# razorx89/nmfgpu

Measured on AMD Instinct MI355X. Metric: NMF MU iterations/sec, dense 10kx5k r=64, higher is better.
Workload: dtype f32; 1 GPU; configs[1]: dense random V 10000x5000, r=64, MU Frobenius, fp32; rows=10000, columns=5000, features=64, error_every=10, parallelism=single GPU

## Files before the change

nmfgpu_amd/csrc/kernels_mu64.hip:

```cpp
#include <hip/hip_runtime.h>
#include <stdint.h>

#include "kernels.h"
#include "split3.h"
#include "gram_image.h"

namespace nmfamd {

typedef float f32x16 __attribute__((ext_vector_type(16)));

template <bool IS_W>
__global__ __launch_bounds__(256) void k_mu64_update(
	float* __restrict__ P, const float* __restrict__ slabs, int S, long slab_stride,
	const float* __restrict__ Q, const float* __restrict__ scale, float eps,
	float* __restrict__ ps, int len_valid, float* __restrict__ gram_partial,
	const float* __restrict__ Gprev, int compute_error, bf16x8* __restrict__ x3_out, int x3_ks) {
	__shared__ __attribute__((aligned(16))) float s_num[64][68];
	__shared__ __attribute__((aligned(16))) float s_old[64][68];
	__shared__ float s_ps[2][64];
	const int tid = threadIdx.x;
	const int wave = tid >> 6, lane = tid & 63;
	const int half = lane >> 5, l31 = lane & 31;
	const int ct = wave & 1, mb = wave >> 1;
	const long tile = (long)blockIdx.x * 64 * 64;
	const int c4 = (4 * tid) & 63;
	const int yl0 = tid >> 4;

	f32x4 nl[4], ol[4];
	{
		f32x4 t[7][4];
#pragma unroll
		for (int j = 0; j < 4; ++j) {
			const long e = tile + 4 * (tid + 256 * j);
			nl[j] = *reinterpret_cast<const f32x4*>(slabs + e);
			ol[j] = *reinterpret_cast<const f32x4*>(P + e);
#pragma unroll
			for (int u = 0; u < 7; ++u) {
				const int k = 1 + u < S ? 1 + u : 0;
				t[u][j] = *reinterpret_cast<const f32x4*>(slabs + (long)k * slab_stride + e);
			}
		}
#pragma unroll
		for (int u = 0; u < 7; ++u)
			if (1 + u < S) {
#pragma unroll
				for (int j = 0; j < 4; ++j) nl[j] += t[u][j];
			}
		for (int k0 = 8; k0 < S; k0 += 7) {
#pragma unroll
			for (int j = 0; j < 4; ++j)
#pragma unroll
				for (int u = 0; u < 7; ++u) {
					const int k = k0 + u < S ? k0 + u : 0;
					t[u][j] = *reinterpret_cast<const f32x4*>(slabs + (long)k * slab_stride + tile + 4 * (tid + 256 * j));
				}
#pragma unroll
			for (int u = 0; u < 7; ++u)
				if (k0 + u < S) {
#pragma unroll
					for (int j = 0; j < 4; ++j) nl[j] += t[u][j];
				}
		}
	}
	const f32x4 sc = *reinterpret_cast<const f32x4*>(scale + c4);
	float qa[32];
#pragma unroll
	for (int cb = 0; cb < 2; ++cb)
#pragma unroll
		for (int q = 0; q < 4; ++q)
#pragma unroll
			for (int gi = 0; gi < 4; ++gi) qa[cb * 16 + q * 4 + gi] = Q[(long)(32 * cb + 8 * q + 4 * half + gi) * 64 + 32 * mb + l31];
#pragma unroll
	for (int j = 0; j < 4; ++j) {
		if (IS_W) ol[j] *= sc; else nl[j] *= sc;
		*reinterpret_cast<f32x4*>(&s_num[yl0 + 16 * j][c4]) = nl[j];
		*reinterpret_cast<f32x4*>(&s_old[yl0 + 16 * j][c4]) = ol[j];
	}
	__syncthreads();

	const int yrow = ct * 32 + l31;
	f32x4 oldv[2][4], numv[4];
#pragma unroll
	for (int cb = 0; cb < 2; ++cb)
#pragma unroll
		for (int q = 0; q < 4; ++q) oldv[cb][q] = *reinterpret_cast<const f32x4*>(&s_old[yrow][32 * cb + 8 * q + 4 * half]);
#pragma unroll
	for (int q = 0; q < 4; ++q) numv[q] = *reinterpret_cast<const f32x4*>(&s_num[yrow][32 * mb + 8 * q + 4 * half]);
	f32x16 acc;
#pragma unroll
	for (int g = 0; g < 16; ++g) acc[g] = 0.f;
#pragma unroll
	for (int cb = 0; cb < 2; ++cb)
#pragma unroll
		for (int q = 0; q < 4; ++q)
#pragma unroll
			for (int gi = 0; gi < 4; ++gi)
				acc = __builtin_amdgcn_mfma_f32_32x32x2f32(qa[cb * 16 + q * 4 + gi], oldv[cb][q][gi], acc, 0, 0, 0);

	float psum = 0.f;
#pragma unroll
	for (int q = 0; q < 4; ++q) {
		f32x4 o;
#pragma unroll
		for (int gi = 0; gi < 4; ++gi) {
			const float old = mb == 0 ? oldv[0][q][gi] : oldv[1][q][gi];
			o[gi] = old * numv[q][gi] / (acc[4 * q + gi] + eps);
			psum += o[gi] * numv[q][gi];
		}
		*reinterpret_cast<f32x4*>(&s_num[yrow][32 * mb + 8 * q + 4 * half]) = o;
	}
	if (!IS_W && compute_error) {
		psum += __shfl_xor(psum, 32);
		if (half == 0) s_ps[mb][yrow] = psum;
	}
	if (IS_W && compute_error && blockIdx.x == 0) {
		for (int d = wave * 16; d < wave * 16 + 16; ++d) {
			float v = Q[(long)lane * 64 + d] * Gprev[(long)d * 64 + lane];
			for (int w = 32; w > 0; w >>= 1) v += __shfl_xor(v, w);
			if (lane == 0) ps[d] = v;
		}
	}
	__syncthreads();
	if (!IS_W && compute_error && tid < 64) {
		const int ycol = blockIdx.x * 64 + tid;
		if (ycol < len_valid) ps[ycol] = s_ps[0][tid] + s_ps[1][tid];
	}

#pragma unroll
	for (int j = 0; j < 4; ++j)
		*reinterpret_cast<f32x4*>(P + tile + 4 * (tid + 256 * j)) = *reinterpret_cast<const f32x4*>(&s_num[yl0 + 16 * j][c4]);
	if (x3_out != nullptr) {
#pragma unroll
		for (int i = 0; i < 2; ++i) {
			const int slot = tid + 256 * i;
			const int r = slot & 31, h = (slot >> 5) & 1, nb = (slot >> 6) & 1, kk = slot >> 7;
			const long ks = 4l * blockIdx.x + kk;
			if (ks < x3_ks) {
				float v[8];
#pragma unroll
				for (int j = 0; j < 8; ++j) {
					const int yl = 16 * kk + 8 * h + j;
					v[j] = blockIdx.x * 64 + yl < len_valid ? s_num[yl][32 * nb + r] : 0.f;
				}
				store_split3(x3_out, ks, 2, nb, h, r, v);
			}
		}
	}
	const int ab = wave >> 1, bb = wave & 1;
	f32x16 g;
#pragma unroll
	for (int i = 0; i < 16; ++i) g[i] = 0.f;
#pragma unroll 8
	for (int x = 0; x < 64; x += 2) {
		const float a = s_num[x + half][ab * 32 + l31];
		const float b = s_num[x + half][bb * 32 + l31];
		g = __builtin_amdgcn_mfma_f32_32x32x2f32(a, b, g, 0, 0, 0);
	}
	float* out = gram_partial + (long)blockIdx.x * 4096;
#pragma unroll
	for (int q = 0; q < 4; ++q)
#pragma unroll
		for (int gi = 0; gi < 4; ++gi) out[(long)(ab * 32 + gi + 8 * q + 4 * half) * 64 + bb * 32 + l31] = g[4 * q + gi];
}

hipError_t launch_mu64_update(int is_w, float* P, const float* slabs, int S, long slab_stride, const float* Q, const float* scale,
                              float eps, float* ps, int len_valid, int len_pad, float* gram_partial, const float* Gprev,
                              int compute_error, hipStream_t stream, void* x3_out, int x3_ks) {
	dim3 grid(len_pad / 64), block(256);
	bf16x8* xo = reinterpret_cast<bf16x8*>(x3_out);
	if (is_w) hipLaunchKernelGGL((k_mu64_update<true>), grid, block, 0, stream, P, slabs, S, slab_stride, Q, scale, eps, ps, len_valid, gram_partial, Gprev, compute_error, xo, x3_ks);
	else hipLaunchKernelGGL((k_mu64_update<false>), grid, block, 0, stream, P, slabs, S, slab_stride, Q, scale, eps, ps, len_valid, gram_partial, Gprev, compute_error, xo, x3_ks);
	return hipGetLastError();
}

#ifndef U32_Q_EARLY
#define U32_Q_EARLY 0
#endif
template <bool IS_W, int U = 7, int QS = 1, bool NS = false>
__global__ __launch_bounds__(256) void k_mu64_update32(
	float* __restrict__ P, const float* __restrict__ slabs, int S, long slab_stride,
	const float* __restrict__ Q, const float* __restrict__ scale, float eps,
	float* __restrict__ ps, int len_valid, const float* __restrict__ Gprev, int compute_error, bf16x8* __restrict__ x3_out, int x3_ks, PeerSlabs peers,
	float* __restrict__ colsq_part, int qsplit, float* __restrict__ q_out, float ns_a_arg, float ns_b_arg, int ns_r) {
	static_assert(!(NS && IS_W), "the smoothing matrix rides the H update only");
	typedef float f32x4v __attribute__((ext_vector_type(4)));
	__shared__ __attribute__((aligned(16))) float s_num[32][68];
	__shared__ __attribute__((aligned(16))) float s_old[32][68];
	__shared__ __attribute__((aligned(16))) float s_sm[NS ? 32 : 1][68];
	__shared__ float s_ps[4][32];
	__shared__ float s_dsum[NS ? 4 : 1][32], s_osum[NS ? 4 : 1][32];
	const float ns_a = NS ? in_vgpr(ns_a_arg) : 1.f, ns_b = NS ? in_vgpr(ns_b_arg) : 0.f;
	const int tid = threadIdx.x;
	const int wave = tid >> 6, lane = tid & 63;
	const int q = lane >> 4, l15 = lane & 15;
	const long tile = (long)blockIdx.x * 32 * 64;
	const int c4 = (4 * tid) & 63;
	const int yl0 = tid >> 4;

	if (peers.count > 0) S = peers.count;
	if (peers.count > 1) __builtin_amdgcn_fence(__ATOMIC_ACQUIRE, "");
	auto slab_at = [&](int k) -> const float* { return peers.count > 0 ? peers.p[k] : slabs + (long)k * slab_stride; };
	f32x4v qa[4];
	f32x4v qs[QS > 1 ? QS - 1 : 1][4];
	f32x4v nl[2], ol[2];
	{
		f32x4v t[U][2];
#pragma unroll
		for (int j = 0; j < 2; ++j) {
			const long e = tile + 4 * (tid + 256 * j);
			nl[j] = *reinterpret_cast<const f32x4v*>(slab_at(0) + e);
			ol[j] = *reinterpret_cast<const f32x4v*>(P + e);
#pragma unroll
			for (int u = 0; u < U; ++u) {
				const int k = 1 + u < S ? 1 + u : 0;
				t[u][j] = *reinterpret_cast<const f32x4v*>(slab_at(k) + e);
			}
		}
		if (QS > 1 || U32_Q_EARLY) {
			__builtin_amdgcn_sched_barrier(0);
#pragma unroll
			for (int u = 0; u < 4; ++u) qa[u] = *reinterpret_cast<const f32x4v*>(Q + (long)(16 * wave + l15) * 64 + 16 * q + 4 * u);
#pragma unroll
			for (int k = 1; k < QS; ++k)
#pragma unroll
				for (int u = 0; u < 4; ++u) qs[k - 1][u] = *reinterpret_cast<const f32x4v*>(Q + (long)k * 4096 + (long)(16 * wave + l15) * 64 + 16 * q + 4 * u);
			__builtin_amdgcn_sched_barrier(0);
		}
#pragma unroll
		for (int u = 0; u < U; ++u)
			if (1 + u < S) {
#pragma unroll
				for (int j = 0; j < 2; ++j) nl[j] += t[u][j];
			}
		for (int k0 = 1 + U; k0 < S; k0 += U) {
#pragma unroll
			for (int j = 0; j < 2; ++j)
#pragma unroll
				for (int u = 0; u < U; ++u) {
					const int k = k0 + u < S ? k0 + u : 0;
					t[u][j] = *reinterpret_cast<const f32x4v*>(slab_at(k) + tile + 4 * (tid + 256 * j));
				}
#pragma unroll
			for (int u = 0; u < U; ++u)
				if (k0 + u < S) {
#pragma unroll
					for (int j = 0; j < 2; ++j) nl[j] += t[u][j];
				}
		}
	}
	const f32x4v sc = *reinterpret_cast<const f32x4v*>(scale + c4);
	if (QS == 1 && !U32_Q_EARLY) {
#pragma unroll
		for (int u = 0; u < 4; ++u) qa[u] = *reinterpret_cast<const f32x4v*>(Q + (long)(16 * wave + l15) * 64 + 16 * q + 4 * u);
	}
	if (!IS_W && QS > 1) {
#pragma unroll
		for (int k = 1; k < QS; ++k)
#pragma unroll
			for (int u = 0; u < 4; ++u) qa[u] += qs[k - 1][u];
		const float srow = scale[16 * wave + l15];
#pragma unroll
		for (int u = 0; u < 4; ++u) {
			const f32x4v scol = *reinterpret_cast<const f32x4v*>(scale + 16 * q + 4 * u);
			qa[u] = (qa[u] * scol) * srow;
			if (blockIdx.x == 0 && q_out != nullptr) *reinterpret_cast<f32x4v*>(q_out + (long)(16 * wave + l15) * 64 + 16 * q + 4 * u) = qa[u];
		}
	}
#pragma unroll
	for (int j = 0; j < 2; ++j) {
		if (IS_W) ol[j] *= sc; else nl[j] *= sc;
		if (NS) {
			float sn = (nl[j][0] + nl[j][1]) + (nl[j][2] + nl[j][3]);
			float so = (ol[j][0] + ol[j][1]) + (ol[j][2] + ol[j][3]);
#pragma unroll
			for (int w = 1; w < 16; w <<= 1) { sn += __shfl_xor(sn, w); so += __shfl_xor(so, w); }
			f32x4v sm;
#pragma unroll
			for (int g = 0; g < 4; ++g) {
				const bool in = c4 + g < ns_r;
				nl[j][g] = in ? ns_a * nl[j][g] + ns_b * sn : 0.f;
				sm[g] = in ? ns_a * ol[j][g] + ns_b * so : 0.f;
			}
			*reinterpret_cast<f32x4v*>(&s_sm[yl0 + 16 * j][c4]) = sm;
		}
		*reinterpret_cast<f32x4v*>(&s_num[yl0 + 16 * j][c4]) = nl[j];
		*reinterpret_cast<f32x4v*>(&s_old[yl0 + 16 * j][c4]) = ol[j];
	}
	__syncthreads();

	f32x4v ob[2][4];
#pragma unroll
	for (int yt = 0; yt < 2; ++yt)
#pragma unroll
		for (int u = 0; u < 4; ++u) ob[yt][u] = *reinterpret_cast<const f32x4v*>(NS ? &s_sm[16 * yt + l15][16 * q + 4 * u] : &s_old[16 * yt + l15][16 * q + 4 * u]);
	f32x4v acc[2] = {{0.f, 0.f, 0.f, 0.f}, {0.f, 0.f, 0.f, 0.f}};
#pragma unroll
	for (int u = 0; u < 4; ++u)
#pragma unroll
		for (int g = 0; g < 4; ++g) {
			acc[0] = __builtin_amdgcn_mfma_f32_16x16x4f32(qa[u][g], ob[0][u][g], acc[0], 0, 0, 0);
			acc[1] = __builtin_amdgcn_mfma_f32_16x16x4f32(qa[u][g], ob[1][u][g], acc[1], 0, 0, 0);
		}
	f32x4v sq = {0.f, 0.f, 0.f, 0.f};
	if (NS) {
#pragma unroll
		for (int yt = 0; yt < 2; ++yt) {
			float v = (acc[yt][0] + acc[yt][1]) + (acc[yt][2] + acc[yt][3]);
			v += __shfl_xor(v, 16);
			v += __shfl_xor(v, 32);
			if (q == 0) s_dsum[wave][16 * yt + l15] = v;
		}
		__syncthreads();
#pragma unroll
		for (int yt = 0; yt < 2; ++yt) {
			const int y = 16 * yt + l15;
			const float tsum = ((s_dsum[0][y] + s_dsum[1][y]) + s_dsum[2][y]) + s_dsum[3][y];
#pragma unroll
			for (int g = 0; g < 4; ++g) acc[yt][g] = ns_a * acc[yt][g] + ns_b * tsum;
		}
	}
#pragma unroll
	for (int yt = 0; yt < 2; ++yt) {
		const int y = 16 * yt + l15;
		const f32x4v oldv = *reinterpret_cast<const f32x4v*>(&s_old[y][16 * wave + 4 * q]);
		const f32x4v numv = *reinterpret_cast<const f32x4v*>(&s_num[y][16 * wave + 4 * q]);
		f32x4v o;
		float psum = 0.f;
#pragma unroll
		for (int g = 0; g < 4; ++g) {
			o[g] = oldv[g] * numv[g] / (acc[yt][g] + eps);
			psum += o[g] * numv[g];
			if (IS_W) sq[g] += o[g] * o[g];
		}
		*reinterpret_cast<f32x4v*>(&s_num[y][16 * wave + 4 * q]) = o;
		if (NS) {
			float v = (o[0] + o[1]) + (o[2] + o[3]);
			v += __shfl_xor(v, 16);
			v += __shfl_xor(v, 32);
			if (q == 0) s_osum[wave][y] = v;
		}
		if (!IS_W && compute_error) {
			psum += __shfl_xor(psum, 16);
			psum += __shfl_xor(psum, 32);
			if (q == 0) s_ps[wave][y] = psum;
		}
	}
	if (IS_W && colsq_part != nullptr) {
#pragma unroll
		for (int g = 0; g < 4; ++g) {
			float v = sq[g];
			v += __shfl_xor(v, 1); v += __shfl_xor(v, 2); v += __shfl_xor(v, 4); v += __shfl_xor(v, 8);
			sq[g] = v;
		}
		if (l15 == 0) *reinterpret_cast<f32x4v*>(colsq_part + (long)blockIdx.x * 64 + 16 * wave + 4 * q) = sq;
	}
	if (IS_W && compute_error && wave == 0) {
		for (int d = blockIdx.x; d < 64; d += gridDim.x) {
			float v = Q[(long)lane * 64 + d] * Gprev[(long)d * 64 + lane];
			for (int w = 32; w > 0; w >>= 1) v += __shfl_xor(v, w);
			if (lane == 0) ps[d] = v;
		}
	}
	__syncthreads();
	if (!IS_W && compute_error && tid < 32) {
		const int ycol = blockIdx.x * 32 + tid;
		if (ycol < len_valid) ps[ycol] = ((s_ps[0][tid] + s_ps[1][tid]) + s_ps[2][tid]) + s_ps[3][tid];
	}
#pragma unroll
	for (int j = 0; j < 2; ++j)
		*reinterpret_cast<f32x4v*>(P + tile + 4 * (tid + 256 * j)) = *reinterpret_cast<const f32x4v*>(&s_num[yl0 + 16 * j][c4]);
	{
		const int r = tid & 31, h = (tid >> 5) & 1, nb = (tid >> 6) & 1, kk = tid >> 7;
		const long ks = 2l * blockIdx.x + kk;
		if (ks < x3_ks) {
			float v[8];
#pragma unroll
			for (int j = 0; j < 8; ++j) {
				const int yl = 16 * kk + 8 * h + j;
				float x = s_num[yl][32 * nb + r];
				if (NS) x = 32 * nb + r < ns_r ? ns_a * x + ns_b * (((s_osum[0][yl] + s_osum[1][yl]) + s_osum[2][yl]) + s_osum[3][yl]) : 0.f;
				v[j] = blockIdx.x * 32 + yl < len_valid ? x : 0.f;
			}
			store_split3(x3_out, ks, 2, nb, h, r, v);
		}
	}
}

template <bool IS_W, int U, int QS, bool NS = false>
static void launch_update32_inst(dim3 grid, hipStream_t stream, float* P, const float* slabs, int S, long slab_stride, const float* Q, const float* scale, float eps, float* ps,
                                 int len_valid, const float* Gprev, int compute_error, bf16x8* xo, int x3_ks, const PeerSlabs& peers, float* colsq_part, float* q_out,
                                 const SmoothAround* ns = nullptr) {
	hipLaunchKernelGGL((k_mu64_update32<IS_W, U, QS, NS>), grid, dim3(256), 0, stream, P, slabs, S, slab_stride, Q, scale, eps, ps, len_valid, Gprev, compute_error, xo, x3_ks, peers,
	                   colsq_part, QS, q_out, NS ? ns->diag - ns->off : 1.f, NS ? ns->off : 0.f, NS ? ns->r : 0);
}

hipError_t launch_mu64_update32(int is_w, float* P, const float* slabs, int S, long slab_stride, const float* Q, const float* scale,
                                float eps, float* ps, int len_valid, int len_pad, const float* Gprev, int compute_error, hipStream_t stream,
                                void* x3_out, int x3_ks, const PeerSlabs* peers, float* colsq_part, int qsplit, float* q_out, const SmoothAround* ns) {
	if (x3_out == nullptr || len_pad % 32 != 0 || (qsplit > 1 && is_w) || (qsplit > 1 && qsplit != 2 && qsplit != 4 && qsplit != 8)) return hipErrorInvalidValue;
	if (ns != nullptr && (is_w || ns->r < 1 || ns->r > 64)) return hipErrorInvalidValue;
	PeerSlabs pa = {};
	if (peers != nullptr) {
		if (peers->count < 1 || peers->count > PEER_SLABS_MAX) return hipErrorInvalidValue;
		pa = *peers;
		S = peers->count;
	}
	dim3 grid(len_pad / 32);
	bf16x8* xo = reinterpret_cast<bf16x8*>(x3_out);
#define NMFAMD_U32(ISW, UU, QQ) launch_update32_inst<ISW, UU, QQ>(grid, stream, P, slabs, S, slab_stride, Q, scale, eps, ps, len_valid, Gprev, compute_error, xo, x3_ks, pa, colsq_part, q_out)
#define NMFAMD_U32NS(UU, QQ) launch_update32_inst<false, UU, QQ, true>(grid, stream, P, slabs, S, slab_stride, Q, scale, eps, ps, len_valid, Gprev, compute_error, xo, x3_ks, pa, colsq_part, q_out, ns)
	if (ns != nullptr) {
		if (S > 8) { if (qsplit == 2) NMFAMD_U32NS(13, 2); else if (qsplit == 4) NMFAMD_U32NS(13, 4); else if (qsplit == 8) NMFAMD_U32NS(13, 8); else NMFAMD_U32NS(13, 1); }
		else { if (qsplit == 2) NMFAMD_U32NS(7, 2); else if (qsplit == 4) NMFAMD_U32NS(7, 4); else if (qsplit == 8) NMFAMD_U32NS(7, 8); else NMFAMD_U32NS(7, 1); }
#undef NMFAMD_U32NS
		return hipGetLastError();
	}
	if (is_w) { if (S > 8) NMFAMD_U32(true, 13, 1); else NMFAMD_U32(true, 7, 1); }
	else if (S > 8) { if (qsplit == 2) NMFAMD_U32(false, 13, 2); else if (qsplit == 4) NMFAMD_U32(false, 13, 4); else if (qsplit == 8) NMFAMD_U32(false, 13, 8); else NMFAMD_U32(false, 13, 1); }
	else { if (qsplit == 2) NMFAMD_U32(false, 7, 2); else if (qsplit == 4) NMFAMD_U32(false, 7, 4); else if (qsplit == 8) NMFAMD_U32(false, 7, 8); else NMFAMD_U32(false, 7, 1); }
#undef NMFAMD_U32
	return hipGetLastError();
}

__global__ __launch_bounds__(256) void k_sum_peers(PeerSlabs src, float* __restrict__ out, int count) {
	__builtin_amdgcn_fence(__ATOMIC_ACQUIRE, "");
	const int i = 4 * (blockIdx.x * 256 + threadIdx.x);
	if (i >= count) return;
	f32x4 s = *reinterpret_cast<const f32x4*>(src.p[0] + i);
	for (int k = 1; k < src.count; ++k) s += *reinterpret_cast<const f32x4*>(src.p[k] + i);
	*reinterpret_cast<f32x4*>(out + i) = s;
}

hipError_t launch_sum_peers(const PeerSlabs& src, float* out, int count, hipStream_t stream) {
	if (src.count < 1 || src.count > PEER_SLABS_MAX || count % 4 != 0) return hipErrorInvalidValue;
	hipLaunchKernelGGL(k_sum_peers, dim3((unsigned)((count / 4 + 255) / 256)), dim3(256), 0, stream, src, out, count);
	return hipGetLastError();
}

__global__ __launch_bounds__(256) void k_gram_image(GramReduceArgs rg) {
	__shared__ __attribute__((aligned(16))) float lds[GRAM_IMAGE_LDS_FLOATS];
	gram_image_block(rg, blockIdx.x, lds);
}

hipError_t launch_gram_image_args(const GramReduceArgs& rg, hipStream_t stream) {
	if (rg.image == nullptr || rg.ksplit > GRAM_KSPLIT_MAX || (rg.ksplit > 1 && rg.normalize != 0 && rg.colsq_part == nullptr)) return hipErrorInvalidValue;
	hipLaunchKernelGGL(k_gram_image, dim3(rg.ksplit > 1 ? GRAM_IMAGE_TILES * rg.ksplit : GRAM_REDUCE_BLOCKS), dim3(256), 0, stream, rg);
	return hipGetLastError();
}

hipError_t launch_gram_from_image(const void* image, int image_ks, float* G, float* scale, int normalize, hipStream_t stream, const float* colsq_part, int colsq_parts) {
	GramReduceArgs rg = {nullptr, 0, G, scale, normalize};
	rg.image = image; rg.image_ks = image_ks;
	rg.colsq_part = colsq_part; rg.colsq_parts = colsq_parts;
	hipLaunchKernelGGL(k_gram_image, dim3(GRAM_REDUCE_BLOCKS), dim3(256), 0, stream, rg);
	return hipGetLastError();
}

__global__ __launch_bounds__(256) void k_mu64_gram_partials(const float* __restrict__ P, float* __restrict__ partial) {
	const int wave = threadIdx.x >> 6, lane = threadIdx.x & 63;
	const int half = lane >> 5, l31 = lane & 31;
	const int ab = wave >> 1, bb = wave & 1;
	const float* p = P + (long)blockIdx.x * 64 * 64;
	f32x16 g;
#pragma unroll
	for (int i = 0; i < 16; ++i) g[i] = 0.f;
#pragma unroll 8
	for (int x = 0; x < 64; x += 2) {
		const float a = p[(long)(x + half) * 64 + ab * 32 + l31];
		const float b = p[(long)(x + half) * 64 + bb * 32 + l31];
		g = __builtin_amdgcn_mfma_f32_32x32x2f32(a, b, g, 0, 0, 0);
	}
	float* out = partial + (long)blockIdx.x * 4096;
#pragma unroll
	for (int q = 0; q < 4; ++q)
#pragma unroll
		for (int gi = 0; gi < 4; ++gi) out[(long)(ab * 32 + gi + 8 * q + 4 * half) * 64 + bb * 32 + l31] = g[4 * q + gi];
}

hipError_t launch_mu64_gram_partials(const float* P, int len_pad, float* partial, hipStream_t stream) {
	hipLaunchKernelGGL(k_mu64_gram_partials, dim3(len_pad / 64), dim3(256), 0, stream, P, partial);
	return hipGetLastError();
}

__global__ __launch_bounds__(512) void k_mu64_gram_reduce(GramReduceArgs rg) {
	__shared__ float lds[64 + 512];
	const int tid = threadIdx.x, blk = blockIdx.x;
	float* s_scale = lds;
	float* s_tmp = lds + 64;
	const int parts = rg.parts;
	if (rg.normalize) {
		if (tid < 128) {
			const int c = tid & 63, g = tid >> 6;
			const int p0 = (parts * g) / 2, p1 = (parts * (g + 1)) / 2;
			float sum = 0.f;
			for (int p = p0; p < p1; p += 8) {
				float v[8];
#pragma unroll
				for (int u = 0; u < 8; ++u) v[u] = rg.partials[(long)(p + u < p1 ? p + u : p0) * 4096 + c * 65];
#pragma unroll
				for (int u = 0; u < 8; ++u)
					if (p + u < p1) sum += v[u];
			}
			s_tmp[g * 64 + c] = sum;
		}
		__syncthreads();
		if (tid < 64) {
			const float d = s_tmp[tid] + s_tmp[64 + tid];
			s_scale[tid] = d > 0.f ? 1.0f / sqrtf(d) : 1.0f;
		}
	} else if (tid < 64) {
		s_scale[tid] = 1.0f;
	}
	__syncthreads();
	{
		const int el = tid & 255, g = tid >> 8;
		const int e = blk * 256 + el;
		const int p0 = (parts * g) / 2, p1 = (parts * (g + 1)) / 2;
		float sum = 0.f;
		for (int p = p0; p < p1; p += 8) {
			float v[8];
#pragma unroll
			for (int u = 0; u < 8; ++u) v[u] = rg.partials[(long)(p + u < p1 ? p + u : p0) * 4096 + e];
#pragma unroll
			for (int u = 0; u < 8; ++u)
				if (p + u < p1) sum += v[u];
		}
		s_tmp[g * 256 + el] = sum;
	}
	__syncthreads();
	if (tid < 256) {
		const int e = blk * 256 + tid;
		const float v = s_tmp[tid] + s_tmp[256 + tid];
		rg.G[e] = (v * s_scale[e & 63]) * s_scale[e >> 6];
	}
	if (blk == 0 && tid < 64 && rg.scale) rg.scale[tid] = s_scale[tid];
}

hipError_t launch_mu64_gram_reduce(const GramReduceArgs& rg, hipStream_t stream) {
	hipLaunchKernelGGL(k_mu64_gram_reduce, dim3(GRAM_REDUCE_BLOCKS), dim3(512), 0, stream, rg);
	return hipGetLastError();
}

__global__ __launch_bounds__(256) void k_scale_gram64(float* __restrict__ G, float* __restrict__ scale) {
	__shared__ float s_scale[64];
	const int tid = threadIdx.x;
	if (tid < 64) {
		const float d = G[tid * 65];
		const float sc = d > 0.f ? 1.0f / sqrtf(d) : 1.0f;
		s_scale[tid] = sc;
		scale[tid] = sc;
	}
	__syncthreads();
	for (int e = tid; e < 4096; e += 256) G[e] = (G[e] * s_scale[e & 63]) * s_scale[e >> 6];
}

hipError_t launch_gram64_from_partials(const float* partials, int parts, float* G, float* scale, hipStream_t stream) {
	hipError_t e = launch_reduce_partials<float>(partials, parts, 4096, G, 4096, stream);
	if (e != hipSuccess || scale == nullptr) return e;
	hipLaunchKernelGGL(k_scale_gram64, dim3(1), dim3(256), 0, stream, G, scale);
	return hipGetLastError();
}

__global__ __launch_bounds__(256) void k_mu64_apply_scale(float* __restrict__ P, long count4, const float* __restrict__ scale) {
	const long e = (long)blockIdx.x * 256 + threadIdx.x;
	if (e >= count4) return;
	f32x4 v = *reinterpret_cast<f32x4*>(P + 4 * e);
	const f32x4 s = *reinterpret_cast<const f32x4*>(scale + (4 * e) % 64);
	v *= s;
	*reinterpret_cast<f32x4*>(P + 4 * e) = v;
}

__global__ __launch_bounds__(256) void k_mu64_apply_scale_x3(float* __restrict__ P, const float* __restrict__ scale, bf16x8* __restrict__ x3_out, int x3_ks) {
	__shared__ __attribute__((aligned(16))) float s_v[16][68];
	const int tid = threadIdx.x;
	const long e = (long)blockIdx.x * 256 + tid;
	f32x4 v = *reinterpret_cast<f32x4*>(P + 4 * e);
	v *= *reinterpret_cast<const f32x4*>(scale + (4 * tid) % 64);
	*reinterpret_cast<f32x4*>(P + 4 * e) = v;
	*reinterpret_cast<f32x4*>(&s_v[tid >> 4][4 * (tid & 15)]) = v;
	__syncthreads();
	if (tid < 128 && (int)blockIdx.x < x3_ks) {
		const int r = tid & 31, h = (tid >> 5) & 1, nb = tid >> 6;
		float w[8];
#pragma unroll
		for (int j = 0; j < 8; ++j) w[j] = s_v[8 * h + j][32 * nb + r];
		store_split3(x3_out, blockIdx.x, 2, nb, h, r, w);
	}
}

__global__ __launch_bounds__(256) void k_mu64_scale_all_x3(float* __restrict__ P, const float* __restrict__ Graw, float* __restrict__ G, float* __restrict__ scale,
                                                          bf16x8* __restrict__ x3_out, int x3_ks, int row_blocks) {
	__shared__ __attribute__((aligned(16))) float s_v[16][68];
	__shared__ __attribute__((aligned(16))) float s_scale[64];
	const int tid = threadIdx.x;
	if (tid < 64) {
		const float d = Graw[tid * 65];
		s_scale[tid] = d > 0.f ? 1.0f / sqrtf(d) : 1.0f;
	}
	__syncthreads();
	if ((int)blockIdx.x == row_blocks) {
		if (tid < 64) scale[tid] = s_scale[tid];
		for (int e = tid; e < 4096; e += 256) G[e] = (Graw[e] * s_scale[e & 63]) * s_scale[e >> 6];
		return;
	}
	const long e = (long)blockIdx.x * 256 + tid;
	f32x4 v = *reinterpret_cast<f32x4*>(P + 4 * e);
	v *= *reinterpret_cast<const f32x4*>(s_scale + (4 * tid) % 64);
	*reinterpret_cast<f32x4*>(P + 4 * e) = v;
	*reinterpret_cast<f32x4*>(&s_v[tid >> 4][4 * (tid & 15)]) = v;
	__syncthreads();
	if (tid < 128 && (int)blockIdx.x < x3_ks) {
		const int r = tid & 31, h = (tid >> 5) & 1, nb = tid >> 6;
		float w[8];
#pragma unroll
		for (int j = 0; j < 8; ++j) w[j] = s_v[8 * h + j][32 * nb + r];
		store_split3(x3_out, blockIdx.x, 2, nb, h, r, w);
	}
}

__global__ __launch_bounds__(256) void k_mu64_reduce_scale_all_x3(float* __restrict__ P, const float* __restrict__ gram_part, int parts, const float* __restrict__ sumsq_part, int sq_parts,
                                                                 float* __restrict__ G, float* __restrict__ scale, bf16x8* __restrict__ x3_out, int x3_ks, int row_blocks) {
	__shared__ __attribute__((aligned(16))) float s_v[16][68];
	__shared__ __attribute__((aligned(16))) float s_scale[64];
	__shared__ float s_grp[4][64];
	const int tid = threadIdx.x;
	{
		const int c = tid & 63, g = tid >> 6;
		float sum = 0.f;
		for (int p = g; p < sq_parts; p += 4 * 48) {
			float v[48];
#pragma unroll
			for (int u = 0; u < 48; ++u) v[u] = p + 4 * u < sq_parts ? sumsq_part[(long)(p + 4 * u) * 64 + c] : 0.f;
#pragma unroll
			for (int u = 0; u < 48; ++u) sum += v[u];
		}
		s_grp[g][c] = sum;
	}
	__syncthreads();
	if (tid < 64) {
		const float d = ((s_grp[0][tid] + s_grp[1][tid]) + s_grp[2][tid]) + s_grp[3][tid];
		s_scale[tid] = d > 0.f ? 1.0f / sqrtf(d) : 1.0f;
	}
	__syncthreads();
	if ((int)blockIdx.x >= row_blocks) {
		const int row = (int)blockIdx.x - row_blocks, c = tid & 63, g = tid >> 6;
		const int p0 = (parts * g) / 4, p1 = (parts * (g + 1)) / 4;
		const float* src = gram_part + (long)row * 64 + c;
		float sum = 0.f;
		for (int p = p0; p < p1; p += 48) {
			float v[48];
#pragma unroll
			for (int u = 0; u < 48; ++u) v[u] = p + u < p1 ? src[(long)(p + u) * 4096] : 0.f;
#pragma unroll
			for (int u = 0; u < 48; ++u) sum += v[u];
		}
		__syncthreads();
		s_grp[g][c] = sum;
		__syncthreads();
		if (tid < 64) {
			const float v = ((s_grp[0][tid] + s_grp[1][tid]) + s_grp[2][tid]) + s_grp[3][tid];
			G[(long)row * 64 + tid] = (v * s_scale[tid]) * s_scale[row];
			if (row == 0) scale[tid] = s_scale[tid];
		}
		return;
	}
	const long e = (long)blockIdx.x * 256 + tid;
	f32x4 v = *reinterpret_cast<f32x4*>(P + 4 * e);
	v *= *reinterpret_cast<const f32x4*>(s_scale + (4 * tid) % 64);
	*reinterpret_cast<f32x4*>(P + 4 * e) = v;
	*reinterpret_cast<f32x4*>(&s_v[tid >> 4][4 * (tid & 15)]) = v;
	__syncthreads();
	if (tid < 128 && (int)blockIdx.x < x3_ks) {
		const int r = tid & 31, h = (tid >> 5) & 1, nb = tid >> 6;
		float w[8];
#pragma unroll
		for (int j = 0; j < 8; ++j) w[j] = s_v[8 * h + j][32 * nb + r];
		store_split3(x3_out, blockIdx.x, 2, nb, h, r, w);
	}
}

hipError_t launch_gram64_reduce_scale_all(const float* gram_part, int parts, const float* sumsq_part, int sq_parts, float* G, float* scale, float* P, int len_pad,
                                          void* x3_out, int x3_ks, hipStream_t stream) {
	if (parts < 1 || sq_parts < 1 || len_pad % 16 != 0) return hipErrorInvalidValue;
	const int row_blocks = len_pad / 16;
	hipLaunchKernelGGL(k_mu64_reduce_scale_all_x3, dim3((unsigned)row_blocks + 64), dim3(256), 0, stream, P, gram_part, parts, sumsq_part, sq_parts, G, scale,
	                   reinterpret_cast<bf16x8*>(x3_out), x3_ks, row_blocks);
	return hipGetLastError();
}

hipError_t launch_gram64_normalize_all(const float* partials, int parts, float* Graw, float* G, float* scale, float* P, int len_pad, void* x3_out, int x3_ks, hipStream_t stream) {
	hipError_t e = launch_reduce_partials<float>(partials, parts, 4096, Graw, 4096, stream);
	if (e != hipSuccess) return e;
	const int row_blocks = len_pad / 16;
	hipLaunchKernelGGL(k_mu64_scale_all_x3, dim3((unsigned)row_blocks + 1), dim3(256), 0, stream, P, Graw, G, scale, reinterpret_cast<bf16x8*>(x3_out), x3_ks, row_blocks);
	return hipGetLastError();
}

hipError_t launch_mu64_apply_scale(float* P, int len_pad, const float* scale, hipStream_t stream, void* x3_out, int x3_ks) {
	if (x3_out != nullptr) {
		hipLaunchKernelGGL(k_mu64_apply_scale_x3, dim3((unsigned)(len_pad / 16)), dim3(256), 0, stream, P, scale, reinterpret_cast<bf16x8*>(x3_out), x3_ks);
		return hipGetLastError();
	}
	const long count4 = (long)len_pad * 64 / 4;
	hipLaunchKernelGGL(k_mu64_apply_scale, dim3((unsigned)((count4 + 255) / 256)), dim3(256), 0, stream, P, count4, scale);
	return hipGetLastError();
}

}
```

Before: 11440 iterations/s.

## Overlap denominator MFMA with slab loads and specialize update kernel per slab count

Restructures the 32-row MU update kernel into two legs. It first loads the old factor tile, Q and scale, stores the old tile to LDS and runs the Q·old MFMA denominator chain while the split-K numerator slab loads are still in flight. Only after that does it sum the slabs and write the numerator to LDS. The launcher also picks a template unroll equal to S-1 for small slab counts, so the batch is exact and the guarded tail loop and redundant clamped loads go away. The cost is more template instantiations, an extra barrier, and higher register pressure from holding the slab loads across the MFMA chain.

```diff
diff --git a/nmfgpu_amd/csrc/kernels_mu64.hip b/nmfgpu_amd/csrc/kernels_mu64.hip
--- a/nmfgpu_amd/csrc/kernels_mu64.hip
+++ b/nmfgpu_amd/csrc/kernels_mu64.hip
@@ -173,9 +173,16 @@
 	return hipGetLastError();
 }
 
+#ifndef U32_EXACT_BATCH
+#define U32_EXACT_BATCH 1
+#endif
+#ifndef U32_TWO_LEG
+#define U32_TWO_LEG 1
+#endif
 #ifndef U32_Q_EARLY
 #define U32_Q_EARLY 0
 #endif
+__device__ __forceinline__ void lds_barrier32() { asm volatile("s_waitcnt lgkmcnt(0)\n\ts_barrier" ::: "memory"); }
 template <bool IS_W, int U = 7, int QS = 1, bool NS = false>
 __global__ __launch_bounds__(256) void k_mu64_update32(
 	float* __restrict__ P, const float* __restrict__ slabs, int S, long slab_stride,
@@ -203,8 +210,126 @@
 	f32x4v qa[4];
 	f32x4v qs[QS > 1 ? QS - 1 : 1][4];
 	f32x4v nl[2], ol[2];
-	{
-		f32x4v t[U][2];
+	constexpr int UB = U > 0 ? U : 1;
+	constexpr bool EXACT = U32_EXACT_BATCH != 0 && U <= 7 && QS == 1 && !NS;
+	f32x4v acc[2] = {{0.f, 0.f, 0.f, 0.f}, {0.f, 0.f, 0.f, 0.f}};
+	auto den_chain = [&]() {
+		f32x4v ob[2][4];
+#pragma unroll
+		for (int yt = 0; yt < 2; ++yt)
+#pragma unroll
+			for (int u = 0; u < 4; ++u) ob[yt][u] = *reinterpret_cast<const f32x4v*>(NS ? &s_sm[16 * yt + l15][16 * q + 4 * u] : &s_old[16 * yt + l15][16 * q + 4 * u]);
+#pragma unroll
+		for (int u = 0; u < 4; ++u)
+#pragma unroll
+			for (int g = 0; g < 4; ++g) {
+				acc[0] = __builtin_amdgcn_mfma_f32_16x16x4f32(qa[u][g], ob[0][u][g], acc[0], 0, 0, 0);
+				acc[1] = __builtin_amdgcn_mfma_f32_16x16x4f32(qa[u][g], ob[1][u][g], acc[1], 0, 0, 0);
+			}
+		if (NS) {
+#pragma unroll
+			for (int yt = 0; yt < 2; ++yt) {
+				float v = (acc[yt][0] + acc[yt][1]) + (acc[yt][2] + acc[yt][3]);
+				v += __shfl_xor(v, 16);
+				v += __shfl_xor(v, 32);
+				if (q == 0) s_dsum[wave][16 * yt + l15] = v;
+			}
+		}
+	};
+	if (U32_TWO_LEG) {
+		f32x4v t[UB][2];
+		f32x4v sc, scol[4];
+		float srow = 1.f;
+#pragma unroll
+		for (int j = 0; j < 2; ++j) ol[j] = *reinterpret_cast<const f32x4v*>(P + tile + 4 * (tid + 256 * j));
+		sc = *reinterpret_cast<const f32x4v*>(scale + c4);
+#pragma unroll
+		for (int u = 0; u < 4; ++u) qa[u] = *reinterpret_cast<const f32x4v*>(Q + (long)(16 * wave + l15) * 64 + 16 * q + 4 * u);
+#pragma unroll
+		for (int k = 1; k < QS; ++k)
+#pragma unroll
+			for (int u = 0; u < 4; ++u) qs[k - 1][u] = *reinterpret_cast<const f32x4v*>(Q + (long)k * 4096 + (long)(16 * wave + l15) * 64 + 16 * q + 4 * u);
+		if (!IS_W && QS > 1) {
+			srow = scale[16 * wave + l15];
+#pragma unroll
+			for (int u = 0; u < 4; ++u) scol[u] = *reinterpret_cast<const f32x4v*>(scale + 16 * q + 4 * u);
+		}
+		__builtin_amdgcn_sched_barrier(0);
+#pragma unroll
+		for (int j = 0; j < 2; ++j) {
+			const long e = tile + 4 * (tid + 256 * j);
+			nl[j] = *reinterpret_cast<const f32x4v*>(slab_at(0) + e);
+#pragma unroll
+			for (int u = 0; u < U; ++u) {
+				const int k = (EXACT || 1 + u < S) ? 1 + u : 0;
+				t[u][j] = *reinterpret_cast<const f32x4v*>(slab_at(k) + e);
+			}
+		}
+		__builtin_amdgcn_sched_barrier(0);
+		if (!IS_W && QS > 1) {
+#pragma unroll
+			for (int k = 1; k < QS; ++k)
+#pragma unroll
+				for (int u = 0; u < 4; ++u) qa[u] += qs[k - 1][u];
+#pragma unroll
+			for (int u = 0; u < 4; ++u) {
+				qa[u] = (qa[u] * scol[u]) * srow;
+				if (blockIdx.x == 0 && q_out != nullptr) *reinterpret_cast<f32x4v*>(q_out + (long)(16 * wave + l15) * 64 + 16 * q + 4 * u) = qa[u];
+			}
+		}
+#pragma unroll
+		for (int j = 0; j < 2; ++j) {
+			if (IS_W) ol[j] *= sc;
+			if (NS) {
+				float so = (ol[j][0] + ol[j][1]) + (ol[j][2] + ol[j][3]);
+#pragma unroll
+				for (int w = 1; w < 16; w <<= 1) so += __shfl_xor(so, w);
+				f32x4v sm;
+#pragma unroll
+				for (int g = 0; g < 4; ++g) sm[g] = c4 + g < ns_r ? ns_a * ol[j][g] + ns_b * so : 0.f;
+				*reinterpret_cast<f32x4v*>(&s_sm[yl0 + 16 * j][c4]) = sm;
+			}
+			*reinterpret_cast<f32x4v*>(&s_old[yl0 + 16 * j][c4]) = ol[j];
+		}
+		lds_barrier32();
+		den_chain();
+		__builtin_amdgcn_sched_barrier(0);
+#pragma unroll
+		for (int u = 0; u < U; ++u)
+			if (EXACT || 1 + u < S) {
+#pragma unroll
+				for (int j = 0; j < 2; ++j) nl[j] += t[u][j];
+			}
+		for (int k0 = 1 + U; !EXACT && k0 < S; k0 += UB) {
+#pragma unroll
+			for (int j = 0; j < 2; ++j)
+#pragma unroll
+				for (int u = 0; u < UB; ++u) {
+					const int k = k0 + u < S ? k0 + u : 0;
+					t[u][j] = *reinterpret_cast<const f32x4v*>(slab_at(k) + tile + 4 * (tid + 256 * j));
+				}
+#pragma unroll
+			for (int u = 0; u < UB; ++u)
+				if (k0 + u < S) {
+#pragma unroll
+					for (int j = 0; j < 2; ++j) nl[j] += t[u][j];
+				}
+		}
+#pragma unroll
+		for (int j = 0; j < 2; ++j) {
+			if (!IS_W) nl[j] *= sc;
+			if (NS) {
+				float sn = (nl[j][0] + nl[j][1]) + (nl[j][2] + nl[j][3]);
+#pragma unroll
+				for (int w = 1; w < 16; w <<= 1) sn += __shfl_xor(sn, w);
+#pragma unroll
+				for (int g = 0; g < 4; ++g) nl[j][g] = c4 + g < ns_r ? ns_a * nl[j][g] + ns_b * sn : 0.f;
+			}
+			*reinterpret_cast<f32x4v*>(&s_num[yl0 + 16 * j][c4]) = nl[j];
+		}
+		__syncthreads();
+	} else {
+		f32x4v t[UB][2];
 #pragma unroll
 		for (int j = 0; j < 2; ++j) {
 			const long e = tile + 4 * (tid + 256 * j);
@@ -212,7 +337,7 @@
 			ol[j] = *reinterpret_cast<const f32x4v*>(P + e);
 #pragma unroll
 			for (int u = 0; u < U; ++u) {
-				const int k = 1 + u < S ? 1 + u : 0;
+				const int k = (EXACT || 1 + u < S) ? 1 + u : 0;
 				t[u][j] = *reinterpret_cast<const f32x4v*>(slab_at(k) + e);
 			}
 		}
@@ -228,89 +353,70 @@
 		}
 #pragma unroll
 		for (int u = 0; u < U; ++u)
-			if (1 + u < S) {
+			if (EXACT || 1 + u < S) {
 #pragma unroll
 				for (int j = 0; j < 2; ++j) nl[j] += t[u][j];
 			}
-		for (int k0 = 1 + U; k0 < S; k0 += U) {
+		for (int k0 = 1 + U; !EXACT && k0 < S; k0 += UB) {
 #pragma unroll
 			for (int j = 0; j < 2; ++j)
 #pragma unroll
-				for (int u = 0; u < U; ++u) {
+				for (int u = 0; u < UB; ++u) {
 					const int k = k0 + u < S ? k0 + u : 0;
 					t[u][j] = *reinterpret_cast<const f32x4v*>(slab_at(k) + tile + 4 * (tid + 256 * j));
 				}
 #pragma unroll
-			for (int u = 0; u < U; ++u)
+			for (int u = 0; u < UB; ++u)
 				if (k0 + u < S) {
 #pragma unroll
 					for (int j = 0; j < 2; ++j) nl[j] += t[u][j];
 				}
 		}
-	}
-	const f32x4v sc = *reinterpret_cast<const f32x4v*>(scale + c4);
-	if (QS == 1 && !U32_Q_EARLY) {
-#pragma unroll
-		for (int u = 0; u < 4; ++u) qa[u] = *reinterpret_cast<const f32x4v*>(Q + (long)(16 * wave + l15) * 64 + 16 * q + 4 * u);
-	}
-	if (!IS_W && QS > 1) {
-#pragma unroll
-		for (int k = 1; k < QS; ++k)
-#pragma unroll
-			for (int u = 0; u < 4; ++u) qa[u] += qs[k - 1][u];
-		const float srow = scale[16 * wave + l15];
-#pragma unroll
-		for (int u = 0; u < 4; ++u) {
-			const f32x4v scol = *reinterpret_cast<const f32x4v*>(scale + 16 * q + 4 * u);
-			qa[u] = (qa[u] * scol) * srow;
-			if (blockIdx.x == 0 && q_out != nullptr) *reinterpret_cast<f32x4v*>(q_out + (long)(16 * wave + l15) * 64 + 16 * q + 4 * u) = qa[u];
-		}
-	}
-#pragma unroll
-	for (int j = 0; j < 2; ++j) {
-		if (IS_W) ol[j] *= sc; else nl[j] *= sc;
-		if (NS) {
-			float sn = (nl[j][0] + nl[j][1]) + (nl[j][2] + nl[j][3]);
-			float so = (ol[j][0] + ol[j][1]) + (ol[j][2] + ol[j][3]);
-#pragma unroll
-			for (int w = 1; w < 16; w <<= 1) { sn += __shfl_xor(sn, w); so += __shfl_xor(so, w); }
-			f32x4v sm;
-#pragma unroll
-			for (int g = 0; g < 4; ++g) {
-				const bool in = c4 + g < ns_r;
-				nl[j][g] = in ? ns_a * nl[j][g] + ns_b * sn : 0.f;
-				sm[g] = in ? ns_a * ol[j][g] + ns_b * so : 0.f;
-			}
-			*reinterpret_cast<f32x4v*>(&s_sm[yl0 + 16 * j][c4]) = sm;
-		}
-		*reinterpret_cast<f32x4v*>(&s_num[yl0 + 16 * j][c4]) = nl[j];
-		*reinterpret_cast<f32x4v*>(&s_old[yl0 + 16 * j][c4]) = ol[j];
-	}
-	__syncthreads();
-
-	f32x4v ob[2][4];
-#pragma unroll
-	for (int yt = 0; yt < 2; ++yt)
-#pragma unroll
-		for (int u = 0; u < 4; ++u) ob[yt][u] = *reinterpret_cast<const f32x4v*>(NS ? &s_sm[16 * yt + l15][16 * q + 4 * u] : &s_old[16 * yt + l15][16 * q + 4 * u]);
-	f32x4v acc[2] = {{0.f, 0.f, 0.f, 0.f}, {0.f, 0.f, 0.f, 0.f}};
-#pragma unroll
-	for (int u = 0; u < 4; ++u)
-#pragma unroll
-		for (int g = 0; g < 4; ++g) {
-			acc[0] = __builtin_amdgcn_mfma_f32_16x16x4f32(qa[u][g], ob[0][u][g], acc[0], 0, 0, 0);
-			acc[1] = __builtin_amdgcn_mfma_f32_16x16x4f32(qa[u][g], ob[1][u][g], acc[1], 0, 0, 0);
-		}
+		const f32x4v sc = *reinterpret_cast<const f32x4v*>(scale + c4);
+		if (QS == 1 && !U32_Q_EARLY) {
+#pragma unroll
+			for (int u = 0; u < 4; ++u) qa[u] = *reinterpret_cast<const f32x4v*>(Q + (long)(16 * wave + l15) * 64 + 16 * q + 4 * u);
+		}
+		if (!IS_W && QS > 1) {
+#pragma unroll
+			for (int k = 1; k < QS; ++k)
+#pragma unroll
+				for (int u = 0; u < 4; ++u) qa[u] += qs[k - 1][u];
+			const float srow = scale[16 * wave + l15];
+#pragma unroll
+			for (int u = 0; u < 4; ++u) {
+				const f32x4v scol = *reinterpret_cast<const f32x4v*>(scale + 16 * q + 4 * u);
+				qa[u] = (qa[u] * scol) * srow;
+				if (blockIdx.x == 0 && q_out != nullptr) *reinterpret_cast<f32x4v*>(q_out + (long)(16 * wave + l15) * 64 + 16 * q + 4 * u) = qa[u];
+			}
+		}
+#pragma unroll
+		for (int j = 0; j < 2; ++j) {
+			if (IS_W) ol[j] *= sc; else nl[j] *= sc;
+			if (NS) {
+				float sn = (nl[j][0] + nl[j][1]) + (nl[j][2] + nl[j][3]);
+				float so = (ol[j][0] + ol[j][1]) + (ol[j][2] + ol[j][3]);
+#pragma unroll
+				for (int w = 1; w < 16; w <<= 1) { sn += __shfl_xor(sn, w); so += __shfl_xor(so, w); }
+				f32x4v sm;
+#pragma unroll
+				for (int g = 0; g < 4; ++g) {
+					const bool in = c4 + g < ns_r;
+					nl[j][g] = in ? ns_a * nl[j][g] + ns_b * sn : 0.f;
+					sm[g] = in ? ns_a * ol[j][g] + ns_b * so : 0.f;
+				}
+				*reinterpret_cast<f32x4v*>(&s_sm[yl0 + 16 * j][c4]) = sm;
+			}
+			*reinterpret_cast<f32x4v*>(&s_num[yl0 + 16 * j][c4]) = nl[j];
+			*reinterpret_cast<f32x4v*>(&s_old[yl0 + 16 * j][c4]) = ol[j];
+		}
+		__syncthreads();
+		den_chain();
+		if (NS) __syncthreads();
+	}
+
 	f32x4v sq = {0.f, 0.f, 0.f, 0.f};
 	if (NS) {
-#pragma unroll
-		for (int yt = 0; yt < 2; ++yt) {
-			float v = (acc[yt][0] + acc[yt][1]) + (acc[yt][2] + acc[yt][3]);
-			v += __shfl_xor(v, 16);
-			v += __shfl_xor(v, 32);
-			if (q == 0) s_dsum[wave][16 * yt + l15] = v;
-		}
-		__syncthreads();
 #pragma unroll
 		for (int yt = 0; yt < 2; ++yt) {
 			const int y = 16 * yt + l15;
@@ -415,9 +521,16 @@
 #undef NMFAMD_U32NS
 		return hipGetLastError();
 	}
-	if (is_w) { if (S > 8) NMFAMD_U32(true, 13, 1); else NMFAMD_U32(true, 7, 1); }
+#define NMFAMD_U32_BY_S(ISW) switch (S) { \
+	case 2: NMFAMD_U32(ISW, 1, 1); break; case 3: NMFAMD_U32(ISW, 2, 1); break; case 4: NMFAMD_U32(ISW, 3, 1); break; case 5: NMFAMD_U32(ISW, 4, 1); break; \
+	case 6: NMFAMD_U32(ISW, 5, 1); break; case 7: NMFAMD_U32(ISW, 6, 1); break; case 8: NMFAMD_U32(ISW, 7, 1); break; \
+	default: if (S > 8) NMFAMD_U32(ISW, 13, 1); else NMFAMD_U32(ISW, 0, 1); break; }
+	if (U32_EXACT_BATCH && is_w) { NMFAMD_U32_BY_S(true); }
+	else if (U32_EXACT_BATCH && qsplit != 2 && qsplit != 4 && qsplit != 8) { NMFAMD_U32_BY_S(false); }
+	else if (is_w) { if (S > 8) NMFAMD_U32(true, 13, 1); else NMFAMD_U32(true, 7, 1); }
 	else if (S > 8) { if (qsplit == 2) NMFAMD_U32(false, 13, 2); else if (qsplit == 4) NMFAMD_U32(false, 13, 4); else if (qsplit == 8) NMFAMD_U32(false, 13, 8); else NMFAMD_U32(false, 13, 1); }
 	else { if (qsplit == 2) NMFAMD_U32(false, 7, 2); else if (qsplit == 4) NMFAMD_U32(false, 7, 4); else if (qsplit == 8) NMFAMD_U32(false, 7, 8); else NMFAMD_U32(false, 7, 1); }
+#undef NMFAMD_U32_BY_S
 #undef NMFAMD_U32
 	return hipGetLastError();
 }
```

Result: faster. 11680 iterations/s (median of 6 runs) (+2.1%).
